# HKUST-Aerial-Robotics/ESVO

Hardware: AMD Instinct MI355X
Metric: mapped events/sec (stereo TS raster + block matching + LM depth refinement + fusion), events resident in HBM before the timed region; exactly K ticks between two synchronisations, i.e. including the fill and the drain of the two-deep tick pipeline (`sustained`: the same workload over 1600 ticks) (higher is better)
Workload: dtype f64

## Files before the change

### esvo_amd/csrc/api_core.hip

```cpp
#include "context.hpp"

namespace esvo_host {
thread_local std::string g_create_error;
}

namespace {

void invert3x3(const double* P, double* Kinv, double* Kinv_t) {
  const double a = P[0], b = P[1], cc = P[2], d = P[4], e = P[5], f = P[6], g = P[8], hh = P[9], i = P[10];
  const double det = a * (e * i - f * hh) - b * (d * i - f * g) + cc * (d * hh - e * g);
  const double id = 1.0 / det;
  Kinv[0] = (e * i - f * hh) * id; Kinv[1] = (cc * hh - b * i) * id; Kinv[2] = (b * f - cc * e) * id;
  Kinv[3] = (f * g - d * i) * id;  Kinv[4] = (a * i - cc * g) * id;  Kinv[5] = (cc * d - a * f) * id;
  Kinv[6] = (d * hh - e * g) * id; Kinv[7] = (b * g - a * hh) * id;  Kinv[8] = (a * e - b * d) * id;
  for (int r = 0; r < 3; ++r) Kinv_t[r] = (Kinv[r * 3 + 0] * P[3] + Kinv[r * 3 + 1] * P[7]) + Kinv[r * 3 + 2] * P[11];
}

int validate_params(const esvo_params_t* p, std::string& why) {
  if (p->ls_norm != ESVO_LSNORM_TDIST && p->ls_norm != ESVO_LSNORM_L2) { why = "LSnorm must be Tdist or l2 (DepthProblemSolver.cpp:121-131 exits on anything else)"; return ESVO_ERR_UNSUPPORTED; }
  if (p->bm_step < 1) { why = "BM_step must be >= 1"; return ESVO_ERR_INVALID_ARG; }
  if (p->patch_size_x < 1 || p->patch_size_x > 64 || p->patch_size_y < 1 || p->patch_size_y > 40) { why = "patch size must be within 1..64 x 1..40"; return ESVO_ERR_UNSUPPORTED; }
  if (p->median_blur_kernel_size < 0 || p->median_blur_kernel_size > 3) { why = "median_blur_kernel_size must be 0..3 (kernel 2k + 1)"; return ESVO_ERR_UNSUPPORTED; }
  if (p->max_event_queue_len < 0 || p->max_event_queue_len > TSQ_LMAX) { why = "max_event_queue_len must be 0 (one stamp per pixel) or 1..32"; return ESVO_ERR_UNSUPPORTED; }
  if (p->bm_max_disparity < p->bm_min_disparity || p->bm_min_disparity < 0) { why = "bad disparity range"; return ESVO_ERR_INVALID_ARG; }
// ... 25 lines not shown
  d.cost_thr = (p.residual_vis_threshold * p.residual_vis_threshold) * (double)(p.patch_size_x * p.patch_size_y);
  d.age_thr = p.age_vis_threshold;
  d.fusion_radius = p.fusion_radius;
  d.reg_radius = p.reg_radius; d.reg_min_nb = p.reg_min_neighbours; d.reg_min_close = p.reg_min_close_neighbours;
  d.num_threads = p.num_threads;
  d.ls_norm = p.ls_norm;
}

template <typename T>
hipError_t dalloc(T** p, size_t n) { return hipMalloc(reinterpret_cast<void**>(p), (n ? n : 1) * sizeof(T)); }

void set_compute_band(esvo_context* h) {
  const int halo = 2 + (h->prm.regularization ? h->prm.reg_radius : 0);
  h->dp.cband_y0 = std::max(0, h->dp.band_y0 - halo);
  h->dp.cband_y1 = std::min(h->H, h->dp.band_y1 + halo);
}

void release_routing(esvo_context* h) {
  for (int cam = 0; cam < 2; ++cam) {
    if (h->h_route_ev[cam]) hipHostFree(h->h_route_ev[cam]);
    h->h_route_ev[cam] = nullptr;
    h->route_cap[cam] = 0;
  }
  if (h->h_route_gidx) hipHostFree(h->h_route_gidx);
  h->h_route_gidx = nullptr;
}

}

extern "C" {
// ... 219 lines not shown
  CK(hipMalloc(reinterpret_cast<void**>(&h->d_map), map_buffer_bytes(npx)));
  CK(hipMalloc(reinterpret_cast<void**>(&h->d_map2), map_buffer_bytes(npx)));
  CK(hipMemset(h->d_map, 0, map_buffer_bytes(npx)));
  CK(hipMemset(h->d_map2, 0, map_buffer_bytes(npx)));
  h->d_map_cur = h->d_map;
  CK(dalloc(&h->d_owner_max, npx));
  CK(dalloc(&h->d_owner_min, npx));
  CK(dalloc(&h->d_own_w, E));
  CK(dalloc(&h->d_lkeep, E));
  h->codes_bytes = (E + 7) / 8 * 8;
  CK(dalloc(&h->d_codes, h->codes_bytes));
  CK(dalloc(&h->d_sel, E));
  CK(dalloc(&h->d_evmap, npx + 64));
  CK(dalloc(&h->d_reg_ab, npx));
  CK(dalloc(&h->d_reg_cd, npx));
  CK(dalloc(&h->d_exp_flags, npx));
  CK(dalloc(&h->d_exp_prefix, npx));
  CK(dalloc(&h->d_export, npx));
  CK(dalloc(&h->d_export_cell, npx));
  for (int i = 0; i < EV_N; ++i) CK(hipEventCreate(&h->evt[i]));
  if (h->tl_on) { CK(hipEventCreate(&h->tl_ref)); CK(hipEventRecord(h->tl_ref, h->stream)); CK(hipEventSynchronize(h->tl_ref)); }
  h->evt_ok = true;
  CK(hipEventCreateWithFlags(&h->evt_trk_read, hipEventDisableTiming));
  for (int cam = 0; cam < 2; ++cam) CK(hipEventCreateWithFlags(&h->evt_ingest[cam], hipEventDisableTiming));
  CK(hipHostMalloc(reinterpret_cast<void**>(&h->h_pose_pool), sizeof(double) * 16 * (size_t)h->max_poses * esvo_context::POSE_POOL));
  for (int i = 0; i < esvo_context::POSE_POOL; ++i) CK(hipEventCreate(&h->pool_evt[i]));
  h->pool_ok = true;
  for (int i = 0; i < 16; ++i) h->T_world_obs[i] = h->T_world_frame[i] = (i % 5 == 0) ? 1.0 : 0.0;
#undef CK
  *out = h;
// ... 4 lines not shown
  if (!h) return ESVO_OK;
  hipSetDevice(h->device);
  if (h->stream) hipStreamSynchronize(h->stream);
  if (h->stream_l) hipStreamSynchronize(h->stream_l);
  if (h->stream_l1) hipStreamSynchronize(h->stream_l1);
  if (h->stream_b) hipStreamSynchronize(h->stream_b);
  comm_release(h);
  em_release(h);
  void* ptrs[] = {h->d_lut, h->d_mask, h->d_fixmap[0], h->d_fixmap[1], h->d_sae[0], h->d_sae[1], h->d_raw, h->d_raw1, h->d_fwd_lut[0], h->d_fwd_lut[1], h->d_fwd_off[0], h->d_fwd_off[1],
                  h->d_fwd_src[0], h->d_fwd_src[1], h->d_fwd_val, h->d_ts[0],
                  h->d_ts[1], h->d_ring[0], h->d_ring[1], h->d_obs2[0][0], h->d_obs2[0][1], h->d_obs2[1][0], h->d_obs2[1][1], h->d_obs_tmp,
                  h->d_pose_T2[0], h->d_pose_T2[1], h->d_scan_tmp_b, h->d_cnt_b, h->d_tick_ev, h->d_match_slots, h->d_match_flags, h->d_match_prefix,
                  h->d_matches2[0], h->d_matches2[1], h->d_scan_tmp_l2[0], h->d_scan_tmp_l2[1], h->d_pt_slots2[0], h->d_pt_slots2[1], h->d_pt_flags2[0], h->d_pt_flags2[1], h->d_pt_prefix2[0], h->d_pt_prefix2[1], h->d_pts_tmp, h->d_stage[0], h->d_stage[1], h->d_counters2[0], h->d_counters2[1], h->d_scan_tmp,
                  h->d_win, h->d_frame_pose_T, h->d_fr_table, h->d_prop, h->d_tile_pts, h->d_tile_count, h->d_over_pts,
                  h->d_cell_count, h->d_cell_offset, h->d_cell_list, h->d_fuse_ctr, h->d_rec_ids, h->d_map, h->d_map2, h->d_owner_max, h->d_owner_min, h->d_exp_flags,
                  h->d_exp_prefix, h->d_export, h->d_export_cell, h->d_reg_ab, h->d_reg_cd, h->d_tsq[0], h->d_tsq[1], h->d_tsq_tcount, h->d_tsq_tlist, h->d_tsq_over, h->d_tsq_over_count, h->d_own_w, h->d_lkeep, h->d_codes, h->d_codes_send, h->d_codes_all, h->d_pts_send, h->d_pts_all, h->d_rank_kept,
                  h->d_sel, h->d_evmap, h->d_lm_fvec0, h->d_lm_fnorm0, h->d_lm_meta, h->d_lm_order, h->d_lm_hist, h->d_clk, h->d_ring_gidx, h->d_halo_viol, h->d_dn_flags, h->d_merge_a, h->d_merge_b, h->d_merge_plan, h->d_tsq_dup};
  for (void* p : ptrs) if (p) hipFree(p);
  if (h->h_counters) hipHostFree(h->h_counters);
  if (h->h_cnt_b) hipHostFree(h->h_cnt_b);
  if (h->h_pin) hipHostFree(h->h_pin);
  if (h->h_fr_table) hipHostFree(h->h_fr_table);
  if (h->evt_ok) for (int i = 0; i < EV_N; ++i) hipEventDestroy(h->evt[i]);
  if (h->pool_ok) for (int i = 0; i < esvo_context::POSE_POOL; ++i) hipEventDestroy(h->pool_evt[i]);
  if (h->h_pose_pool) hipHostFree(h->h_pose_pool);
  if (h->h_trk_ne) hipHostFree(h->h_trk_ne);
  if (h->h_trk_solve) hipHostFree(h->h_trk_solve);
  if (h->h_trk_xyz) hipHostFree(h->h_trk_xyz);
  release_routing(h);
  for (int cam = 0; cam < 2; ++cam) if (h->d_wire[cam]) hipFree(h->d_wire[cam]);
  if (h->evt_trk_read) hipEventDestroy(h->evt_trk_read);
// ... 118 lines not shown
    if (need > h->max_frames) FAIL(ESVO_ERR_CAPACITY, "fusion window (frames) exceeds the capacity fixed at esvo_create");
  }
  if (h->routed && (params->smooth_time_surface != h->prm.smooth_time_surface || params->median_blur_kernel_size != h->prm.median_blur_kernel_size ||
                    params->patch_size_y != h->prm.patch_size_y || params->denoising != h->prm.denoising || params->bm_updown))
    FAIL(ESVO_ERR_STATE, "the handle routes events by row (esvo_shard_set_routing): SmoothTimeSurface, median_blur_kernel_size, patch_size_Y and Denoising "
                         "fix the rows it renders and the events it keeps; esvo_reset + esvo_shard_set_routing to change them");
  esvo_params_t np = *params;
  np.max_events_per_tick = h->prm.max_events_per_tick;
  np.max_window_points = h->prm.max_window_points;
  np.max_poses_per_tick = h->prm.max_poses_per_tick;
  np.event_ring_capacity = h->prm.event_ring_capacity;
  if (np.max_event_queue_len != h->prm.max_event_queue_len) FAIL(ESVO_ERR_CAPACITY, "max_event_queue_len is fixed at esvo_create (the per-pixel queues are allocated there)");
  h->prm = np;
  fill_dev_params(h);
  set_compute_band(h);
  return ESVO_OK;
}

int esvo_set_stream(esvo_handle h, void* hip_stream) {
  if (!h) return ESVO_ERR_INVALID_ARG;
  API_LOCK(h);
  std::lock_guard<std::mutex> lp0(h->mu_push[0]), lp1(h->mu_push[1]);
  { int rcp = flush_pending_tick(h); if (rcp) return rcp; }
  HIPCHK(hipStreamSynchronize(h->stream));
  HIPCHK(hipStreamSynchronize(h->stream_l)); HIPCHK(hipStreamSynchronize(h->stream_l1));
  HIPCHK(hipStreamSynchronize(h->stream_b));
  if (h->own_stream && h->stream) hipStreamDestroy(h->stream);
  h->stream = reinterpret_cast<hipStream_t>(hip_stream);
  h->own_stream = false;
  return ESVO_OK;
// ... 105 lines not shown
```

### esvo_amd/csrc/api_map.hip

```cpp
#include <chrono>

#include "context.hpp"

namespace esvo_host {

u64 lower_bound_sec(const esvo_context* h, int cam, double t) {
  const auto& v = h->ts_host[cam];
  size_t lo = 0, hi = v.size();
  while (lo < hi) {
    size_t mid = (lo + hi) / 2;
    if (ns_to_sec(v[mid]) < t) lo = mid + 1; else hi = mid;
  }
  return h->ring_base[cam] + lo;
}
u64 ros_time_from_sec(double t) {
  long long sec64 = (long long)std::floor(t);
  u32 sec = (u32)sec64;
  u32 nsec = (u32)std::round((t - sec) * 1e9);
  sec += (nsec / 1000000000ul);
  nsec %= 1000000000ul;
  return (u64)sec * 1000000000ull + nsec;
}

int upload_poses(esvo_context* h, const uint64_t* pose_t_ns, const double* pose_T, size_t m, u32* d_zero_row = nullptr) {
// ... 351 lines not shown
  const int o = par * EV_BACK_STRIDE;
  const bool timed = h->stage_events_on;
  h->back_timed[par] = timed;
  if (timed) hipEventRecord(h->evt[EV_FU0 + o], sb);
  launch_fuse(a, h->dp, sb);
  if (timed) hipEventRecord(h->evt[EV_FU1 + o], sb);
  h->d_map_cur = h->d_map;
  h->map_id_bound = total * ((naive || h->dp.fusion_radius == 0) ? 4u : 9u);
  const bool do_clean = naive ? false : (h->prm.clean_requires_full_window ? (h->n_window_frames >= (size_t)h->prm.max_fusion_frames) : true);
  if (do_clean) launch_clean(h->d_map, h->dp, sb);
  if (timed) hipEventRecord(h->evt[EV_CL1 + o], sb);
  if (h->prm.regularization && !naive) {
    launch_reg_view(h->d_map, h->d_map2, h->d_owner_max, h->d_owner_min, h->d_reg_ab, h->d_reg_cd, h->d_cnt_b + 7, h->dp, sb);
    const u64 band_cells = (u64)std::max(h->dp.band_y1 - h->dp.band_y0, 1) * (u64)h->W;
    const bool sparse = h->reg_sparse_forced >= 0 ? h->reg_sparse_forced == 1 : (u64)h->stats.last_map_size * 10u < band_cells;
    launch_reg_apply(h->d_map, h->d_map2, h->d_owner_max, h->d_owner_min, h->d_reg_ab, h->d_reg_cd, h->d_cnt_b + 7, h->dp, sb, sparse);
    h->d_map_cur = h->d_map2;
  }
  HIPCHK(hipMemcpyAsync(h->h_cnt_b + 8 * par, h->d_cnt_b, sizeof(u32) * 8, hipMemcpyDeviceToHost, sb));
  if (h->routed) HIPCHK(hipMemcpyAsync(h->h_cnt_b + 8 * 3 + par, h->d_halo_viol, sizeof(u32), hipMemcpyDeviceToHost, sb));
  hipEventRecord(h->evt[EV_RG1 + o], sb);
  for (int e : tail_ev) if (e >= 0) hipEventRecord(h->evt[e], sb);
  HIPCHK(hipGetLastError());
  h->back_pending[par] = true;
  return ESVO_OK;
}

int export_map(esvo_context* h, std::vector<esvo_depth_point_t>& out, std::vector<u32>* cells) {
  launch_map_compact(h->d_map_cur, h->d_exp_flags, h->d_exp_prefix, h->d_cnt_b + 5, h->d_scan_tmp_b, h->d_export,
                     h->d_export_cell, h->dp, h->stream_b);
  int rc = read_counters_b(h, 2, true);
// ... 1653 lines not shown
```

### esvo_amd/csrc/common.hpp

```cpp
#pragma once

#include <hip/hip_runtime.h>
#include <stdint.h>

#include "../../include/esvo_hip.h"

#define ESVO_WAVE 64

#include <cstdlib>
#include <cstring>
inline const char* esvo_dev_switch(const char* name) {
  const char* on = std::getenv("ESVO_DEV_SWITCHES");
  return (on && std::strcmp(on, "1") == 0) ? std::getenv(name) : nullptr;
}

namespace esvo {

typedef unsigned long long u64;
typedef unsigned int u32;

struct CamConst {
  double P[12];
  double Kinv[9];
  double Kinv_t[3];
// ... 301 lines not shown
  u32 lds_cap;
  u32 pmax_plus1;
  u32* d_total;
  MapCell* map;
  u32* d_num_fusion;
  u32* n_touched;
  int naive;
  u32* owner_max;
  u32* owner_min;
  u32* n_reg_elems;
};
void launch_fuse(const FuseArgs& a, const DevParams& p, hipStream_t s);
void launch_clean(MapCell* map, const DevParams& p, hipStream_t s);
void launch_reg_view(const MapCell* map_in, MapCell* map_out, u32* owner_max, u32* owner_min, double2* ab, double2* cd,
                     u32* n_elems, const DevParams& p, hipStream_t s);
void launch_reg_apply(const MapCell* map_in, MapCell* map_out, const u32* owner_max, const u32* owner_min, const double2* ab,
                      const double2* cd, u32* n_elems, const DevParams& p, hipStream_t s, bool sparse = false);
struct SgmScratch {
  uint8_t *sobL, *rawL, *sobR, *rawR;
  int16_t* vol[6];
  int16_t *d1, *d1b;
  u32* d2key;
};
void launch_sgbm(const uint8_t* left, const uint8_t* right, const SgmScratch& s, int16_t* disp, int W, int H, hipStream_t st);
void launch_sgm_points(const esvo_event_t* ring, u64 first, u64 cap, u32 n, const float2* lut, const int16_t* disp, DevPoint* slots,
                       u32* flags, const DevParams& p, hipStream_t st);
void launch_sgm_tick_points(const esvo_event_t* ev, u64 first, u64 cap, int reverse, u32 n, const float2* lut, const int16_t* disp,
                            DevPoint* slots, u32* flags, u32* cnt, const DevParams& p, hipStream_t st);
void launch_sgm_naive(const DevPoint* pts, u32 n, const double* d_T_frame_obs, u32* owner, u32* pair_flags, u32* pair_rank, u32* d_total,
                      u32* scan_tmp, MapCell* map, const DevParams& p, hipStream_t st);
void launch_debug_image(const MapCell* map, u32* owner, uint8_t* bgr, const uint8_t* jet, int type, double max_range,
                        double min_range, double thr1, double thr2, const DevParams& p, hipStream_t s);
// ... 7 lines not shown
```

### esvo_amd/csrc/context.hpp

```cpp
#pragma once
#include <algorithm>
#include <array>
#include <atomic>
#include <chrono>
#include <cmath>
#include <cstdio>
#include <cstdlib>
#include <cstring>
#include <deque>
#include <mutex>
#include <string>
#include <vector>

#include "common.hpp"

using namespace esvo;

enum { EV_SC0 = 0, EV_SC1, EV_R1, EV_SC0b, EV_SC1b, EV_R1b, EV_FRAME,
       EV_T0, EV_BM0, EV_BM1, EV_S1, EV_LM0, EV_LM1, EV_S2, EV_CNT, EV_STG, EV_A1, EV_T0b, EV_BM0b, EV_BM1b, EV_S1b, EV_LM0b, EV_LM1b, EV_S2b, EV_CNTb, EV_STGb, EV_A1b,
       EV_FU0, EV_FU1, EV_CL1, EV_RG1, EV_POSE, EV_FU0b, EV_FU1b, EV_CL1b, EV_RG1b, EV_POSEb, EV_N };
constexpr int EV_BACK_STRIDE = EV_FU0b - EV_FU0;
constexpr int EV_FRONT_STRIDE = EV_T0b - EV_T0;
constexpr int EV_TS_STRIDE = EV_SC0b - EV_SC0;

// ... 241 lines not shown
  bool tick_pending = false;
  u64 committed_t_ns = 0;
  int tsq_len = 0;
  u64* d_tsq[2] = {nullptr, nullptr};
  u32* d_tsq_tcount = nullptr;
  uint4* d_tsq_tlist = nullptr;
  uint4* d_tsq_over = nullptr;
  u32* d_tsq_over_count = nullptr;
  u32 tsq_tcap = 0;
  static constexpr u64 TSQ_ROUND = 1ull << 20;
  u64 sh_first = 0;
  u64 sh_first_prev = 0;
  u64 em_guard_lo[2] = {~0ull, ~0ull};
  double2* d_reg_ab = nullptr;
  double2* d_reg_cd = nullptr;
  double T_world_frame[16];
  u32* d_exp_flags = nullptr;
  u32* d_exp_prefix = nullptr;
  esvo_depth_point_t* d_export = nullptr;
  u32* d_export_cell = nullptr;
  u32 map_id_bound = 0;
  float* d_cloud_xyz[2] = {nullptr, nullptr};
  int cloud_cur = -1;
  size_t cloud_n = 0;
  u64 cloud_t_ns = 0;
  u32* d_cloud_ids = nullptr;
  size_t cloud_id_cap = 0;
  u32* d_cloud_scan = nullptr;
  u32* d_cloud_cnt = nullptr;
  u32* h_cloud_cnt = nullptr;
// ... 146 lines not shown
```

### esvo_amd/csrc/dev_hooks.hpp

```cpp
#pragma once
#if defined(LM_STATS) || defined(REG_STATS) || defined(ESVO_PERTURB_ONE_ULP)
#include "../../tools/dev_hooks/hooks_impl.hpp"
#endif
#ifndef LM_STATS
#define DEV_LM_EVAL(pr) do {} while (0)
#define DEV_LM_SHORTCUT(pr) do {} while (0)
#define DEV_LM_PROBLEM_FIELDS
#define DEV_LM_SET_SLOT(pr, s) do {} while (0)
#define DEV_LM_FIRST_EVAL_KNZ(pr, knz) do {} while (0)
#define DEV_LM_SCALE_ITER(pr) do {} while (0)
#define DEV_LM_JAC_DECL
#define DEV_LM_JAC_PASS(pr, active, x) do {} while (0)
#endif
#ifndef ESVO_PERTURB_ONE_ULP
#define DEV_PERTURB_POINT(o, s) do {} while (0)
#endif
#ifndef REG_STATS
#define DEV_REG_DECL
#define DEV_REG_BLOCK_BEGIN() do {} while (0)
#define DEV_REG_ROW_BEGIN(nclose)
#define DEV_REG_ROW_END(nclose) do {} while (0)
#define DEV_REG_BLOCK_END(lane, wv) do {} while (0)
#define DEV_REG_DONE(t, lane, nclose) do {} while (0)
#endif
```

### esvo_amd/csrc/kernels_fuse.hip

```cpp
#include <algorithm>
#include <type_traits>
#define DEV_HOOKS_FUSE_TU
#include "common.hpp"
#include "dev_hooks.hpp"
#include "fdiv.hpp"
#include "scan.hpp"

namespace esvo {

#ifndef BACK_WAVES
#define BACK_WAVES 6
#endif
#ifndef FUSE_WAVES
#define FUSE_WAVES 1
#endif

__device__ inline bool boundaryCheck(double x, double y, int W, int H) {
  return !(x < 0 || x >= (double)W || y < 0 || y >= (double)H);
}

__device__ inline bool fusion_cell(u32 prow, u32 pcol, int k, int radius, int W, int H, int& row, int& col) {
  int dy, dx;
  if (radius == 0) { dy = k >> 1; dx = k & 1; }
  else { dy = k / 3 - 1; dx = k % 3 - 1; }
// ... 624 lines not shown
  }
  const u64 am = __ballot(alive);
  if (n_elems && (threadIdx.x & 63) == 0 && am) atomicAdd(n_elems, (u32)__popcll(am));
}

#define REG_TX 64
#ifndef REG_TY
#define REG_TY 8
#endif
#ifndef REG_RB
#define REG_RB 4
#endif
#define REG_MARGIN 1
#define REG_MAXW 128
static_assert((REG_TX * REG_TY) % 64 == 0 && REG_TX == 64, "a wave is a tile row");
template <int RT, bool SPARSE = false>
__global__ void __launch_bounds__(REG_TX * REG_TY, BACK_WAVES) reg_apply_kernel(const MapCell* __restrict__ map, MapCell* __restrict__ out,
                                                                    const u32* __restrict__ owner_max,
                                                                    const u32* __restrict__ owner_min,
                                                                    const double2* __restrict__ ab,
                                                                    const double2* __restrict__ cd, DevParams p, u32* __restrict__ n_elems) {
  constexpr int NW = REG_TY;
  constexpr int UNITS = 4 * REG_RB;
  constexpr int UPW = (UNITS + NW - 1) / NW;
  __shared__ double2 s_ab[2][REG_RB][REG_MAXW];
  __shared__ double2 s_cd[2][REG_RB][REG_MAXW];
  __shared__ u64 s_vb[2][REG_RB][2];
  __shared__ u32 s_elem[REG_TX * REG_TY];
  __shared__ u32 s_wcount[REG_TY + 1];
  const int t = threadIdx.x, lane = t & 63, wv = t >> 6;
  const int tiles_x = (p.W + REG_TX - 1) / REG_TX;
  const int tile_c0 = (int)(blockIdx.x % tiles_x) * REG_TX, tile_r0 = (int)(blockIdx.x / tiles_x) * REG_TY;
  const int R = RT > 0 ? RT : p.reg_radius, Wn = 2 * R + 1;
  const int cr = tile_r0 + wv, cc = tile_c0 + lane;
  bool alive = false;
  if (cr < p.H && cc < p.W && cr >= p.band_y0 && cr < p.band_y1) alive = (map_flags(map, p.W * p.H)[cr * p.W + cc] & CELL_ALIVE) != 0;
  const u64 am = __ballot(alive);
  if (lane == 0) s_wcount[wv] = (u32)__popcll(am);
  __syncthreads();
  u32 base = 0, n_el = 0;
  for (int w = 0; w < REG_TY; ++w) { if (w < wv) base += s_wcount[w]; n_el += s_wcount[w]; }
  if (n_el == 0) return;
  if (t == 0) atomicAdd(n_elems, n_el);
  if (alive) s_elem[base + (u32)__popcll(am & ((1ull << lane) - 1ull))] = (u32)(cr * p.W + cc);
  __syncthreads();
  const bool has = (u32)t < n_el;
  int cell = 0, row = 0, col = 0;
  double inv = -1.0, sd_self2 = 0.0;
  u32 seq = 0;
  if (has) {
    cell = (int)s_elem[t];
    const MapCell& c = map[cell];
    row = (int)c.row; col = (int)c.col;
    inv = c.inv_depth;
    sd_self2 = 2.0 * sqrt(c.variance);
    seq = c.seq;
  }
  const u32 b = (u32)row * (u32)p.W + (u32)col;
  const bool owner = has && owner_max[b] == seq + 1u;
  bool scan = owner && inv > -1e-6 && row >= R && col >= R;
  const int sc0 = tile_c0 - REG_MARGIN - R, sr0 = tile_r0 - REG_MARGIN - R;
  const int sw = REG_TX + 2 * (R + REG_MARGIN), sh = REG_TY + 2 * (R + REG_MARGIN);
  const int off = col - R - sc0;
  bool slow = scan && (off < 0 || off + Wn > sw || row - R < sr0 || row + R >= sr0 + sh);
  if (slow) scan = false;
  const u64 wmask = (Wn >= 64) ? ~0ull : ((1ull << Wn) - 1ull);
  u32 nb = 0, nclose = 0;
  double nu_post = 0, inv_post = 0, s2_post = 0, nu_div = 0;
  Recip rnu = make_recip(1.0);
  bool first = true;
  auto fuse_step = [&](double inv_obs, double nu_obs, double s2_obs) {
    if (first) {
      first = false;
      nu_post = nu_obs; inv_post = inv_obs; s2_post = s2_obs;
      nu_div = nu_post + 1;
      rnu = make_recip(nu_div);
      return;
    }
    const double nu_prior = nu_post, inv_prior = inv_post, s2_prior = s2_post;
    nu_post = (nu_obs < nu_prior) ? nu_obs : nu_prior;
    if (nu_post + 1 != nu_div) { nu_div = nu_post + 1; rnu = make_recip(nu_div); }
    const double ssum = s2_obs + s2_prior;
    const Recip rsum = make_recip(ssum);
    const double a1 = s2_obs * inv_prior + s2_prior * inv_obs;
    const double dd = inv_prior - inv_obs;
    const double a2 = dd * dd;
    const double pp = s2_prior * s2_obs;
    const double q1 = div_fast(a1, rsum);
    const double a3 = nu_post + div_fast(a2, rsum);
    const double a4 = div_fast(a3, rnu) * pp;
    const double q4 = div_fast(a4, rsum);
    const bool ok = (int)rnu.fast & (int)fdiv_ok_b4(ssum, a1, a2, a3, a4);
    if (ok) {
      inv_post = q1;
      s2_post = q4;
    } else {
      inv_post = a1 / ssum;
      s2_post = ((nu_post + a2 / ssum) / (nu_post + 1) * pp) / ssum;
    }
  };
  const double nan = __longlong_as_double(0x7ff8000000000000ll);
  double2 ld[UPW];
  const int n_blk = (sh + REG_RB - 1) / REG_RB;
  auto fetch_block = [&](int k) {
#pragma unroll
    for (int j = 0; j < UPW; ++j) {
      const int u = wv + NW * j;
      ld[j] = make_double2(nan, nan);
      if (u < UNITS && k < n_blk) {
        const int r = u >> 2, a = (u >> 1) & 1, hf = u & 1;
        const int y = k * REG_RB + r, sj = hf * 64 + lane;
        const int gy = sr0 + y, gx = sc0 + sj;
        if (sj < sw && y < sh && gy >= 0 && gy < p.H && gx >= 0 && gx < p.W) ld[j] = (a ? cd : ab)[gy * p.W + gx];
      }
    }
  };
  auto store_block = [&](int buf) {
#pragma unroll
    for (int j = 0; j < UPW; ++j) {
      const int u = wv + NW * j;
      if (u < UNITS) {
        const int r = u >> 2, a = (u >> 1) & 1, hf = u & 1;
        const int sj = hf * 64 + lane;
        (a ? s_cd : s_ab)[buf][r][sj] = ld[j];
        if (!a) {
          const u64 vm = __ballot(sj < sw && ld[j].x == ld[j].x);
          if (lane == 0) s_vb[buf][r][hf] = vm;
        }
      }
    }
  };
  DEV_REG_DECL
  fetch_block(0);
  store_block(0);
  fetch_block(1);
  __syncthreads();
  for (int k = 0; k < n_blk; ++k) {
    const int buf = k & 1;
    DEV_REG_BLOCK_BEGIN();
#pragma unroll 1
    for (int r = 0; r < REG_RB; ++r) {
      const int gy = sr0 + k * REG_RB + r;
      DEV_REG_ROW_BEGIN(nclose)
      if (scan && gy >= row - R && gy <= row + R) {
        const u64 w0 = s_vb[buf][r][0], w1 = s_vb[buf][r][1];
        u64 bits = (off < 64) ? (w0 >> off) : 0ull;
        if (off > 0 && off < 64) bits |= w1 << (64 - off);
        if (off >= 64) bits = w1 >> (off - 64);
        bits &= wmask;
        nb += (u32)__popcll(bits);
        u32 cm2[2] = {0u, 0u};
        if (bits) {
          u32 lo = 0, hi = 0;
          const double2* tap = &s_ab[buf][r][off];
          if constexpr (SPARSE) {
#pragma unroll 1
            for (int half = 0; half < 2; ++half) {
              u32 m = half ? (u32)(bits >> 32) : (u32)bits;
              u32 acc = 0;
              while (m) {
                const int kk = __builtin_ctz(m);
                m &= m - 1u;
                const double2 q = tap[32 * half + kk];
                acc |= (fabs(inv - q.x) < fmax(sd_self2, q.y)) ? (1u << kk) : 0u;
              }
              if (half) hi = acc; else lo = acc;
            }
          } else if (RT > 0) {
#pragma unroll
            for (int dc = 0; dc < 2 * RT + 1; ++dc) {
              const double2 q = tap[dc];
              const bool close = fabs(inv - q.x) < fmax(sd_self2, q.y);
              if (dc < 32) lo |= close ? (1u << dc) : 0u; else hi |= close ? (1u << (dc - 32)) : 0u;
            }
          } else {
            for (int dc = 0; dc < Wn; ++dc) {
              const double2 q = tap[dc];
              const bool close = fabs(inv - q.x) < fmax(sd_self2, q.y);
              if (dc < 32) lo |= close ? (1u << dc) : 0u; else hi |= close ? (1u << (dc - 32)) : 0u;
            }
          }
          cm2[0] = lo; cm2[1] = hi;
        }
        nclose += (u32)__popc(cm2[0]) + (u32)__popc(cm2[1]);
#pragma unroll 1
        for (int half = 0; half < 2; ++half) {
          u32 m = half ? cm2[1] : cm2[0];
          const int o2 = off + 32 * half;
          while (m) {
            const int kk = __builtin_ctz(m);
            m &= m - 1u;
            const double2 qa = s_ab[buf][r][o2 + kk], qc = s_cd[buf][r][o2 + kk];
            fuse_step(qa.x, qc.x, qc.y);
          }
        }
      }
      DEV_REG_ROW_END(nclose);
    }
    DEV_REG_BLOCK_END(lane, wv);
    if (k + 1 < n_blk) store_block(buf ^ 1);
    fetch_block(k + 2);
    __syncthreads();
  }
  DEV_REG_DONE(t, lane, nclose);
  if (slow) {
    for (int r = row - R; r <= row + R && r < p.H; ++r)
      for (int c2 = col - R; c2 <= col + R && c2 < p.W; ++c2) {
        const double2 q = ab[r * p.W + c2];
        if (!(q.x == q.x)) continue;
        nb++;
        const double diff = fabs(inv - q.x);
        if (diff < sd_self2 || diff < q.y) {
          nclose++;
          const double2 qc = cd[r * p.W + c2];
          fuse_step(q.x, qc.x, qc.y);
        }
      }
  }
  if (!has) return;
  u32* of = map_flags(out, p.W * p.H);
  if (!owner) { of[cell] = 0; return; }
  MapCell c = map[cell];
  if (c.inv_depth > -1e-6)
    c.inv_depth = (nb > (u32)p.reg_min_nb && nclose > (u32)p.reg_min_close) ? inv_post : -1.0;
  c.seq = owner_min[b];
  out[cell] = c;
  of[cell] = CELL_ALIVE | CELL_GRID;
}

__global__ void __launch_bounds__(256) reg_apply_l2_kernel(const MapCell* __restrict__ map, MapCell* __restrict__ out,
                                                           const u32* __restrict__ owner_max, const u32* __restrict__ owner_min,
                                                           const double2* __restrict__ ab, const double2* __restrict__ cd, DevParams p) {
  const int cell = blockIdx.x * blockDim.x + threadIdx.x;
  if (cell >= p.W * p.H) return;
  { const int r0 = cell / p.W; if (r0 < p.band_y0 || r0 >= p.band_y1) return; }
  if (!(map_flags(map, p.W * p.H)[cell] & CELL_ALIVE)) return;
  MapCell c = map[cell];
  u32* of = map_flags(out, p.W * p.H);
  const int row = (int)c.row, col = (int)c.col, R = p.reg_radius;
  const u32 b = (u32)row * (u32)p.W + (u32)col;
  if (owner_max[b] != c.seq + 1u) { of[cell] = 0; return; }
  if (c.inv_depth > -1e-6) {
// ... 23 lines not shown
    c.inv_depth = set ? mean : -1.0;
  }
  c.seq = owner_min[b];
  out[cell] = c;
  of[cell] = CELL_ALIVE | CELL_GRID;
}

void launch_reg_view(const MapCell* map_in, MapCell* map_out, u32* owner_max, u32* owner_min, double2* ab, double2* cd,
                     u32* n_elems, const DevParams& p, hipStream_t s) {
  const int ncell = p.W * p.H;
  const int nb = (ncell + 255) / 256;
  if (p.ls_norm != ESVO_LSNORM_L2) n_elems = nullptr;
  hipLaunchKernelGGL(reg_view_kernel, dim3(nb), dim3(256), 0, s, map_in, map_out, ab, cd, owner_max, owner_min, n_elems, ncell, p.W,
                     p.band_y0, p.band_y1, p.cband_y0, p.cband_y1, p.ls_norm == ESVO_LSNORM_L2 ? 1 : 0);
}
void launch_reg_apply(const MapCell* map_in, MapCell* map_out, const u32* owner_max, const u32* owner_min, const double2* ab,
                      const double2* cd, u32* n_elems, const DevParams& p, hipStream_t s, bool sparse) {
  if (p.ls_norm == ESVO_LSNORM_L2) {
    const int ncell = p.W * p.H;
    hipLaunchKernelGGL(reg_apply_l2_kernel, dim3((ncell + 255) / 256), dim3(256), 0, s, map_in, map_out, owner_max, owner_min, ab, cd, p);
    return;
  }
  const int tiles_x = (p.W + REG_TX - 1) / REG_TX;
  const int ty0 = p.band_y0 / REG_TY, ty1 = (p.band_y1 + REG_TY - 1) / REG_TY;
  if (ty1 <= ty0) return;
  const int tiles_y = (p.H + REG_TY - 1) / REG_TY;
  const dim3 grid(tiles_x * tiles_y), block(REG_TX * REG_TY);
  if (sparse) {
    if (p.reg_radius == 20) hipLaunchKernelGGL((reg_apply_kernel<20, true>), grid, block, 0, s, map_in, map_out, owner_max, owner_min, ab, cd, p, n_elems);
    else if (p.reg_radius == 5) hipLaunchKernelGGL((reg_apply_kernel<5, true>), grid, block, 0, s, map_in, map_out, owner_max, owner_min, ab, cd, p, n_elems);
    else hipLaunchKernelGGL((reg_apply_kernel<0, true>), grid, block, 0, s, map_in, map_out, owner_max, owner_min, ab, cd, p, n_elems);
    return;
  }
  if (p.reg_radius == 20) hipLaunchKernelGGL(reg_apply_kernel<20>, grid, block, 0, s, map_in, map_out, owner_max, owner_min, ab, cd, p, n_elems);
  else if (p.reg_radius == 5) hipLaunchKernelGGL(reg_apply_kernel<5>, grid, block, 0, s, map_in, map_out, owner_max, owner_min, ab, cd, p, n_elems);
  else hipLaunchKernelGGL(reg_apply_kernel<0>, grid, block, 0, s, map_in, map_out, owner_max, owner_min, ab, cd, p, n_elems);
}

__global__ void __launch_bounds__(256) map_flags_kernel(const MapCell* __restrict__ map, u32* __restrict__ flags, int ncell, int W,
                                                        int band0, int band1) {
  const int cell = blockIdx.x * blockDim.x + threadIdx.x;
  if (cell >= ncell) return;
  const int row = cell / W;
  flags[cell] = (row >= band0 && row < band1 && (map_flags(map, ncell)[cell] & CELL_ALIVE)) ? 1u : 0u;
}
__global__ void __launch_bounds__(256) map_export_kernel(const MapCell* __restrict__ map, const u32* __restrict__ flags,
                                                         const u32* __restrict__ prefix, esvo_depth_point_t* __restrict__ out,
                                                         u32* __restrict__ out_cell, int ncell) {
  const int cell = blockIdx.x * blockDim.x + threadIdx.x;
  if (cell >= ncell || !flags[cell]) return;
  const MapCell& c = map[cell];
// ... 21 lines not shown
```

Measured before the change: 154.4 million.

## Split regularisation into mask scan plus load-balanced sorted fusion walk kernel

The regularisation apply kernel now only computes per-row close-neighbour bitmasks and writes them to a per-cell record buffer. It then buckets cells by neighbour count into class/slice lists. A new turn kernel prefix-sums the class counts, and a walk kernel assigns one lane per cell, ordered by workload class, to run the sequential fusion steps with a small prefetch queue. This targets wave divergence in the serial fuse loop, where cells with very different neighbour counts shared a wave and the cd tile also had to be staged in LDS. The cost is extra kernel launches, global record traffic and more scratch memory.

```diff
diff --git a/esvo_amd/csrc/api_core.hip b/esvo_amd/csrc/api_core.hip
--- a/esvo_amd/csrc/api_core.hip
+++ b/esvo_amd/csrc/api_core.hip
@@ -63,6 +63,31 @@
   const int halo = 2 + (h->prm.regularization ? h->prm.reg_radius : 0);
   h->dp.cband_y0 = std::max(0, h->dp.band_y0 - halo);
   h->dp.cband_y1 = std::min(h->H, h->dp.band_y1 + halo);
+}
+
+hipError_t reg_walk_alloc(esvo_context* h) {
+  RegWalk& w = h->reg_walk;
+  if (!h->prm.regularization) return hipSuccess;
+  const size_t npx = (size_t)h->W * h->H;
+  hipError_t e;
+  if (!w.list) {
+    w.cap = (u32)npx;
+    w.slice_cap = reg_slice_cap(h->W, h->H);
+    if ((e = dalloc(&w.list, (size_t)REG_NB * REG_SLICES * w.slice_cap)) != hipSuccess) return e;
+    if ((e = dalloc(&w.class_count, 2 * (size_t)REG_NB * REG_SLICES + 1)) != hipSuccess) return e;
+    if ((e = hipMemset(w.class_count, 0, sizeof(u32) * (2 * (size_t)REG_NB * REG_SLICES + 1))) != hipSuccess) return e;
+    w.class_total = w.class_count + REG_NB * REG_SLICES;
+  }
+  const u32 words = reg_rec_words(h->prm.reg_radius);
+  if (words > h->reg_rec_alloc_words) {
+    if (h->stream_b && (e = hipStreamSynchronize(h->stream_b)) != hipSuccess) return e;
+    if (w.rec) { hipFree(w.rec); w.rec = nullptr; h->reg_rec_alloc_words = 0; }
+    if ((e = dalloc(&w.rec, npx * words)) != hipSuccess) return e;
+    h->reg_rec_alloc_words = words;
+  }
+  w.rec_words = words;
+  w.class_width = reg_class_width(h->prm.reg_radius);
+  return hipSuccess;
 }
 
 void release_routing(esvo_context* h) {
@@ -312,6 +337,7 @@
   CK(dalloc(&h->d_evmap, npx + 64));
   CK(dalloc(&h->d_reg_ab, npx));
   CK(dalloc(&h->d_reg_cd, npx));
+  CK(reg_walk_alloc(h));
   CK(dalloc(&h->d_exp_flags, npx));
   CK(dalloc(&h->d_exp_prefix, npx));
   CK(dalloc(&h->d_export, npx));
@@ -346,7 +372,7 @@
                   h->d_matches2[0], h->d_matches2[1], h->d_scan_tmp_l2[0], h->d_scan_tmp_l2[1], h->d_pt_slots2[0], h->d_pt_slots2[1], h->d_pt_flags2[0], h->d_pt_flags2[1], h->d_pt_prefix2[0], h->d_pt_prefix2[1], h->d_pts_tmp, h->d_stage[0], h->d_stage[1], h->d_counters2[0], h->d_counters2[1], h->d_scan_tmp,
                   h->d_win, h->d_frame_pose_T, h->d_fr_table, h->d_prop, h->d_tile_pts, h->d_tile_count, h->d_over_pts,
                   h->d_cell_count, h->d_cell_offset, h->d_cell_list, h->d_fuse_ctr, h->d_rec_ids, h->d_map, h->d_map2, h->d_owner_max, h->d_owner_min, h->d_exp_flags,
-                  h->d_exp_prefix, h->d_export, h->d_export_cell, h->d_reg_ab, h->d_reg_cd, h->d_tsq[0], h->d_tsq[1], h->d_tsq_tcount, h->d_tsq_tlist, h->d_tsq_over, h->d_tsq_over_count, h->d_own_w, h->d_lkeep, h->d_codes, h->d_codes_send, h->d_codes_all, h->d_pts_send, h->d_pts_all, h->d_rank_kept,
+                  h->d_exp_prefix, h->d_export, h->d_export_cell, h->d_reg_ab, h->d_reg_cd, h->reg_walk.rec, h->reg_walk.list, h->reg_walk.class_count, h->d_tsq[0], h->d_tsq[1], h->d_tsq_tcount, h->d_tsq_tlist, h->d_tsq_over, h->d_tsq_over_count, h->d_own_w, h->d_lkeep, h->d_codes, h->d_codes_send, h->d_codes_all, h->d_pts_send, h->d_pts_all, h->d_rank_kept,
                   h->d_sel, h->d_evmap, h->d_lm_fvec0, h->d_lm_fnorm0, h->d_lm_meta, h->d_lm_order, h->d_lm_hist, h->d_clk, h->d_ring_gidx, h->d_halo_viol, h->d_dn_flags, h->d_merge_a, h->d_merge_b, h->d_merge_plan, h->d_tsq_dup};
   for (void* p : ptrs) if (p) hipFree(p);
   if (h->h_counters) hipHostFree(h->h_counters);
@@ -495,6 +521,7 @@
   h->prm = np;
   fill_dev_params(h);
   set_compute_band(h);
+  HIPCHK(reg_walk_alloc(h));
   return ESVO_OK;
 }
 
diff --git a/esvo_amd/csrc/api_map.hip b/esvo_amd/csrc/api_map.hip
--- a/esvo_amd/csrc/api_map.hip
+++ b/esvo_amd/csrc/api_map.hip
@@ -389,7 +389,7 @@
     launch_reg_view(h->d_map, h->d_map2, h->d_owner_max, h->d_owner_min, h->d_reg_ab, h->d_reg_cd, h->d_cnt_b + 7, h->dp, sb);
     const u64 band_cells = (u64)std::max(h->dp.band_y1 - h->dp.band_y0, 1) * (u64)h->W;
     const bool sparse = h->reg_sparse_forced >= 0 ? h->reg_sparse_forced == 1 : (u64)h->stats.last_map_size * 10u < band_cells;
-    launch_reg_apply(h->d_map, h->d_map2, h->d_owner_max, h->d_owner_min, h->d_reg_ab, h->d_reg_cd, h->d_cnt_b + 7, h->dp, sb, sparse);
+    launch_reg_apply(h->d_map, h->d_map2, h->d_owner_max, h->d_owner_min, h->d_reg_ab, h->d_reg_cd, h->d_cnt_b + 7, h->dp, sb, sparse, h->reg_walk);
     h->d_map_cur = h->d_map2;
   }
   HIPCHK(hipMemcpyAsync(h->h_cnt_b + 8 * par, h->d_cnt_b, sizeof(u32) * 8, hipMemcpyDeviceToHost, sb));
diff --git a/esvo_amd/csrc/common.hpp b/esvo_amd/csrc/common.hpp
--- a/esvo_amd/csrc/common.hpp
+++ b/esvo_amd/csrc/common.hpp
@@ -339,8 +339,23 @@
 void launch_clean(MapCell* map, const DevParams& p, hipStream_t s);
 void launch_reg_view(const MapCell* map_in, MapCell* map_out, u32* owner_max, u32* owner_min, double2* ab, double2* cd,
                      u32* n_elems, const DevParams& p, hipStream_t s);
+#define REG_NB 16
+#define REG_SLICES 16
+struct RegWalk {
+  u32* rec;
+  u32 rec_words;
+  u32 cap;
+  u32* list;
+  u32 slice_cap;
+  u32 class_width;
+  u32* class_count;
+  u32* class_total;
+};
+__host__ __device__ inline u32 reg_rec_words(int radius) { return 2u + 2u * (2u * (u32)radius + 1u); }
+__host__ __device__ inline u32 reg_class_width(int radius) { const u32 wn = 2u * (u32)radius + 1u; const u32 w = wn * wn / 70u; return w < 4u ? 4u : w; }
+u32 reg_slice_cap(int W, int H);
 void launch_reg_apply(const MapCell* map_in, MapCell* map_out, const u32* owner_max, const u32* owner_min, const double2* ab,
-                      const double2* cd, u32* n_elems, const DevParams& p, hipStream_t s, bool sparse = false);
+                      const double2* cd, u32* n_elems, const DevParams& p, hipStream_t s, bool sparse, const RegWalk& w);
 struct SgmScratch {
   uint8_t *sobL, *rawL, *sobR, *rawR;
   int16_t* vol[6];
diff --git a/esvo_amd/csrc/context.hpp b/esvo_amd/csrc/context.hpp
--- a/esvo_amd/csrc/context.hpp
+++ b/esvo_amd/csrc/context.hpp
@@ -279,6 +279,8 @@
   u64 em_guard_lo[2] = {~0ull, ~0ull};
   double2* d_reg_ab = nullptr;
   double2* d_reg_cd = nullptr;
+  RegWalk reg_walk{};
+  u32 reg_rec_alloc_words = 0;
   double T_world_frame[16];
   u32* d_exp_flags = nullptr;
   u32* d_exp_prefix = nullptr;
diff --git a/esvo_amd/csrc/dev_hooks.hpp b/esvo_amd/csrc/dev_hooks.hpp
--- a/esvo_amd/csrc/dev_hooks.hpp
+++ b/esvo_amd/csrc/dev_hooks.hpp
@@ -16,10 +16,6 @@
 #define DEV_PERTURB_POINT(o, s) do {} while (0)
 #endif
 #ifndef REG_STATS
-#define DEV_REG_DECL
-#define DEV_REG_BLOCK_BEGIN() do {} while (0)
-#define DEV_REG_ROW_BEGIN(nclose)
-#define DEV_REG_ROW_END(nclose) do {} while (0)
-#define DEV_REG_BLOCK_END(lane, wv) do {} while (0)
-#define DEV_REG_DONE(t, lane, nclose) do {} while (0)
+#define DEV_REG_SCAN_DONE(walk, nclose) do {} while (0)
+#define DEV_REG_WALK_DONE(lane, has, n) do {} while (0)
 #endif
diff --git a/esvo_amd/csrc/kernels_fuse.hip b/esvo_amd/csrc/kernels_fuse.hip
--- a/esvo_amd/csrc/kernels_fuse.hip
+++ b/esvo_amd/csrc/kernels_fuse.hip
@@ -662,62 +662,11 @@
 #define REG_MARGIN 1
 #define REG_MAXW 128
 static_assert((REG_TX * REG_TY) % 64 == 0 && REG_TX == 64, "a wave is a tile row");
-template <int RT, bool SPARSE = false>
-__global__ void __launch_bounds__(REG_TX * REG_TY, BACK_WAVES) reg_apply_kernel(const MapCell* __restrict__ map, MapCell* __restrict__ out,
-                                                                    const u32* __restrict__ owner_max,
-                                                                    const u32* __restrict__ owner_min,
-                                                                    const double2* __restrict__ ab,
-                                                                    const double2* __restrict__ cd, DevParams p, u32* __restrict__ n_elems) {
-  constexpr int NW = REG_TY;
-  constexpr int UNITS = 4 * REG_RB;
-  constexpr int UPW = (UNITS + NW - 1) / NW;
-  __shared__ double2 s_ab[2][REG_RB][REG_MAXW];
-  __shared__ double2 s_cd[2][REG_RB][REG_MAXW];
-  __shared__ u64 s_vb[2][REG_RB][2];
-  __shared__ u32 s_elem[REG_TX * REG_TY];
-  __shared__ u32 s_wcount[REG_TY + 1];
-  const int t = threadIdx.x, lane = t & 63, wv = t >> 6;
-  const int tiles_x = (p.W + REG_TX - 1) / REG_TX;
-  const int tile_c0 = (int)(blockIdx.x % tiles_x) * REG_TX, tile_r0 = (int)(blockIdx.x / tiles_x) * REG_TY;
-  const int R = RT > 0 ? RT : p.reg_radius, Wn = 2 * R + 1;
-  const int cr = tile_r0 + wv, cc = tile_c0 + lane;
-  bool alive = false;
-  if (cr < p.H && cc < p.W && cr >= p.band_y0 && cr < p.band_y1) alive = (map_flags(map, p.W * p.H)[cr * p.W + cc] & CELL_ALIVE) != 0;
-  const u64 am = __ballot(alive);
-  if (lane == 0) s_wcount[wv] = (u32)__popcll(am);
-  __syncthreads();
-  u32 base = 0, n_el = 0;
-  for (int w = 0; w < REG_TY; ++w) { if (w < wv) base += s_wcount[w]; n_el += s_wcount[w]; }
-  if (n_el == 0) return;
-  if (t == 0) atomicAdd(n_elems, n_el);
-  if (alive) s_elem[base + (u32)__popcll(am & ((1ull << lane) - 1ull))] = (u32)(cr * p.W + cc);
-  __syncthreads();
-  const bool has = (u32)t < n_el;
-  int cell = 0, row = 0, col = 0;
-  double inv = -1.0, sd_self2 = 0.0;
-  u32 seq = 0;
-  if (has) {
-    cell = (int)s_elem[t];
-    const MapCell& c = map[cell];
-    row = (int)c.row; col = (int)c.col;
-    inv = c.inv_depth;
-    sd_self2 = 2.0 * sqrt(c.variance);
-    seq = c.seq;
-  }
-  const u32 b = (u32)row * (u32)p.W + (u32)col;
-  const bool owner = has && owner_max[b] == seq + 1u;
-  bool scan = owner && inv > -1e-6 && row >= R && col >= R;
-  const int sc0 = tile_c0 - REG_MARGIN - R, sr0 = tile_r0 - REG_MARGIN - R;
-  const int sw = REG_TX + 2 * (R + REG_MARGIN), sh = REG_TY + 2 * (R + REG_MARGIN);
-  const int off = col - R - sc0;
-  bool slow = scan && (off < 0 || off + Wn > sw || row - R < sr0 || row + R >= sr0 + sh);
-  if (slow) scan = false;
-  const u64 wmask = (Wn >= 64) ? ~0ull : ((1ull << Wn) - 1ull);
-  u32 nb = 0, nclose = 0;
+struct RegFuse {
   double nu_post = 0, inv_post = 0, s2_post = 0, nu_div = 0;
   Recip rnu = make_recip(1.0);
   bool first = true;
-  auto fuse_step = [&](double inv_obs, double nu_obs, double s2_obs) {
+  __device__ inline void step(double inv_obs, double nu_obs, double s2_obs) {
     if (first) {
       first = false;
       nu_post = nu_obs; inv_post = inv_obs; s2_post = s2_obs;
@@ -746,7 +695,62 @@
       inv_post = a1 / ssum;
       s2_post = ((nu_post + a2 / ssum) / (nu_post + 1) * pp) / ssum;
     }
-  };
+  }
+};
+template <int RT, bool SPARSE = false>
+__global__ void __launch_bounds__(REG_TX * REG_TY, BACK_WAVES) reg_apply_kernel(const MapCell* __restrict__ map, MapCell* __restrict__ out,
+                                                                    const u32* __restrict__ owner_max,
+                                                                    const u32* __restrict__ owner_min,
+                                                                    const double2* __restrict__ ab,
+                                                                    const double2* __restrict__ cd, DevParams p, u32* __restrict__ n_elems, RegWalk w) {
+  constexpr int NW = REG_TY;
+  constexpr int UNITS = 2 * REG_RB;
+  constexpr int UPW = (UNITS + NW - 1) / NW;
+  __shared__ double2 s_ab[2][REG_RB][REG_MAXW];
+  __shared__ u64 s_vb[2][REG_RB][2];
+  __shared__ u32 s_elem[REG_TX * REG_TY];
+  __shared__ u32 s_wcount[REG_TY + 1];
+  __shared__ u32 s_hist[REG_NB], s_hbase[REG_NB];
+  const int t = threadIdx.x, lane = t & 63, wv = t >> 6;
+  const int tiles_x = (p.W + REG_TX - 1) / REG_TX;
+  const int tile_c0 = (int)(blockIdx.x % tiles_x) * REG_TX, tile_r0 = (int)(blockIdx.x / tiles_x) * REG_TY;
+  const int R = RT > 0 ? RT : p.reg_radius, Wn = 2 * R + 1;
+  const int cr = tile_r0 + wv, cc = tile_c0 + lane;
+  bool alive = false;
+  if (cr < p.H && cc < p.W && cr >= p.band_y0 && cr < p.band_y1) alive = (map_flags(map, p.W * p.H)[cr * p.W + cc] & CELL_ALIVE) != 0;
+  const u64 am = __ballot(alive);
+  if (lane == 0) s_wcount[wv] = (u32)__popcll(am);
+  if (t < REG_NB) s_hist[t] = 0;
+  __syncthreads();
+  u32 base = 0, n_el = 0;
+  for (int w = 0; w < REG_TY; ++w) { if (w < wv) base += s_wcount[w]; n_el += s_wcount[w]; }
+  if (n_el == 0) return;
+  if (t == 0) s_wcount[REG_TY] = atomicAdd(n_elems, n_el);
+  if (alive) s_elem[base + (u32)__popcll(am & ((1ull << lane) - 1ull))] = (u32)(cr * p.W + cc);
+  __syncthreads();
+  const bool has = (u32)t < n_el;
+  int cell = 0, row = 0, col = 0;
+  double inv = -1.0, sd_self2 = 0.0;
+  u32 seq = 0;
+  if (has) {
+    cell = (int)s_elem[t];
+    const MapCell& c = map[cell];
+    row = (int)c.row; col = (int)c.col;
+    inv = c.inv_depth;
+    sd_self2 = 2.0 * sqrt(c.variance);
+    seq = c.seq;
+  }
+  const u32 b = (u32)row * (u32)p.W + (u32)col;
+  const bool owner = has && owner_max[b] == seq + 1u;
+  bool scan = owner && inv > -1e-6 && row >= R && col >= R;
+  const int sc0 = tile_c0 - REG_MARGIN - R, sr0 = tile_r0 - REG_MARGIN - R;
+  const int sw = REG_TX + 2 * (R + REG_MARGIN), sh = REG_TY + 2 * (R + REG_MARGIN);
+  const int off = col - R - sc0;
+  const u32 slot = s_wcount[REG_TY] + (u32)t;
+  bool slow = scan && (off < 0 || off + Wn > sw || row - R < sr0 || row + R >= sr0 + sh || slot >= w.cap);
+  if (slow) scan = false;
+  const u64 wmask = (Wn >= 64) ? ~0ull : ((1ull << Wn) - 1ull);
+  u32 nb = 0, nclose = 0;
   const double nan = __longlong_as_double(0x7ff8000000000000ll);
   double2 ld[UPW];
   const int n_blk = (sh + REG_RB - 1) / REG_RB;
@@ -756,10 +760,10 @@
       const int u = wv + NW * j;
       ld[j] = make_double2(nan, nan);
       if (u < UNITS && k < n_blk) {
-        const int r = u >> 2, a = (u >> 1) & 1, hf = u & 1;
+        const int r = u >> 1, hf = u & 1;
         const int y = k * REG_RB + r, sj = hf * 64 + lane;
         const int gy = sr0 + y, gx = sc0 + sj;
-        if (sj < sw && y < sh && gy >= 0 && gy < p.H && gx >= 0 && gx < p.W) ld[j] = (a ? cd : ab)[gy * p.W + gx];
+        if (sj < sw && y < sh && gy >= 0 && gy < p.H && gx >= 0 && gx < p.W) ld[j] = ab[gy * p.W + gx];
       }
     }
   };
@@ -768,28 +772,23 @@
     for (int j = 0; j < UPW; ++j) {
       const int u = wv + NW * j;
       if (u < UNITS) {
-        const int r = u >> 2, a = (u >> 1) & 1, hf = u & 1;
+        const int r = u >> 1, hf = u & 1;
         const int sj = hf * 64 + lane;
-        (a ? s_cd : s_ab)[buf][r][sj] = ld[j];
-        if (!a) {
-          const u64 vm = __ballot(sj < sw && ld[j].x == ld[j].x);
-          if (lane == 0) s_vb[buf][r][hf] = vm;
-        }
+        s_ab[buf][r][sj] = ld[j];
+        const u64 vm = __ballot(sj < sw && ld[j].x == ld[j].x);
+        if (lane == 0) s_vb[buf][r][hf] = vm;
       }
     }
   };
-  DEV_REG_DECL
   fetch_block(0);
   store_block(0);
   fetch_block(1);
   __syncthreads();
   for (int k = 0; k < n_blk; ++k) {
     const int buf = k & 1;
-    DEV_REG_BLOCK_BEGIN();
 #pragma unroll 1
     for (int r = 0; r < REG_RB; ++r) {
       const int gy = sr0 + k * REG_RB + r;
-      DEV_REG_ROW_BEGIN(nclose)
       if (scan && gy >= row - R && gy <= row + R) {
         const u64 w0 = s_vb[buf][r][0], w1 = s_vb[buf][r][1];
         u64 bits = (off < 64) ? (w0 >> off) : 0ull;
@@ -819,7 +818,9 @@
             for (int dc = 0; dc < 2 * RT + 1; ++dc) {
               const double2 q = tap[dc];
               const bool close = fabs(inv - q.x) < fmax(sd_self2, q.y);
-              if (dc < 32) lo |= close ? (1u << dc) : 0u; else hi |= close ? (1u << (dc - 32)) : 0u;
+              u32 c01 = close ? 1u : 0u;
+              asm volatile("" : "+v"(c01));
+              if (dc < 32) lo |= c01 << dc; else hi |= c01 << (dc - 32);
             }
           } else {
             for (int dc = 0; dc < Wn; ++dc) {
@@ -831,27 +832,16 @@
           cm2[0] = lo; cm2[1] = hi;
         }
         nclose += (u32)__popc(cm2[0]) + (u32)__popc(cm2[1]);
-#pragma unroll 1
-        for (int half = 0; half < 2; ++half) {
-          u32 m = half ? cm2[1] : cm2[0];
-          const int o2 = off + 32 * half;
-          while (m) {
-            const int kk = __builtin_ctz(m);
-            m &= m - 1u;
-            const double2 qa = s_ab[buf][r][o2 + kk], qc = s_cd[buf][r][o2 + kk];
-            fuse_step(qa.x, qc.x, qc.y);
-          }
-        }
-      }
-      DEV_REG_ROW_END(nclose);
-    }
-    DEV_REG_BLOCK_END(lane, wv);
+        *reinterpret_cast<uint2*>(w.rec + (size_t)slot * w.rec_words + (2 + 2 * (gy - (row - R)))) = make_uint2(cm2[0], cm2[1]);
+      }
+    }
     if (k + 1 < n_blk) store_block(buf ^ 1);
     fetch_block(k + 2);
     __syncthreads();
   }
-  DEV_REG_DONE(t, lane, nclose);
+  double inv_plain = 0.0;
   if (slow) {
+    RegFuse f;
     for (int r = row - R; r <= row + R && r < p.H; ++r)
       for (int c2 = col - R; c2 <= col + R && c2 < p.W; ++c2) {
         const double2 q = ab[r * p.W + c2];
@@ -861,19 +851,138 @@
         if (diff < sd_self2 || diff < q.y) {
           nclose++;
           const double2 qc = cd[r * p.W + c2];
-          fuse_step(q.x, qc.x, qc.y);
+          f.step(q.x, qc.x, qc.y);
         }
       }
-  }
-  if (!has) return;
+    inv_plain = f.inv_post;
+  }
+  cell = has ? (int)s_elem[t] : 0;
+  const u32 slot_e = s_wcount[REG_TY] + (u32)t;
+  const bool keep = nb > (u32)p.reg_min_nb && nclose > (u32)p.reg_min_close;
+  const bool walk = scan && keep;
+  DEV_REG_SCAN_DONE(walk, nclose);
+  u32 cls = 0, rank = 0;
+  if (walk) {
+    cls = nclose / w.class_width;
+    cls = cls < REG_NB - 1u ? cls : REG_NB - 1u;
+    rank = atomicAdd(&s_hist[cls], 1u);
+    *reinterpret_cast<uint2*>(w.rec + (size_t)slot_e * w.rec_words) = make_uint2((u32)cell, nclose);
+  }
+  __syncthreads();
+  const u32 slice = blockIdx.x % REG_SLICES;
+  if (t < REG_NB && s_hist[t]) s_hbase[t] = atomicAdd(&w.class_count[t * REG_SLICES + slice], s_hist[t]);
+  __syncthreads();
+  if (walk) w.list[((size_t)cls * REG_SLICES + slice) * w.slice_cap + s_hbase[cls] + rank] = slot_e;
+  if (!has || walk) return;
   u32* of = map_flags(out, p.W * p.H);
   if (!owner) { of[cell] = 0; return; }
   MapCell c = map[cell];
   if (c.inv_depth > -1e-6)
-    c.inv_depth = (nb > (u32)p.reg_min_nb && nclose > (u32)p.reg_min_close) ? inv_post : -1.0;
-  c.seq = owner_min[b];
+    c.inv_depth = keep ? inv_plain : -1.0;
+  c.seq = owner_min[(u32)row * (u32)p.W + (u32)col];
   out[cell] = c;
   of[cell] = CELL_ALIVE | CELL_GRID;
+}
+
+#define REG_NSEG (REG_NB * REG_SLICES)
+__global__ void __launch_bounds__(REG_NSEG) reg_turn_kernel(RegWalk w) {
+  __shared__ u32 lds[REG_NSEG / ESVO_WAVE];
+  const u32 seg = threadIdx.x;
+  const u32 cls = REG_NB - 1u - seg / REG_SLICES, slc = seg % REG_SLICES;
+  const u32 c = w.class_count[cls * REG_SLICES + slc];
+  w.class_count[cls * REG_SLICES + slc] = 0;
+  u32 tot;
+  const u32 ex = block_excl_scan<REG_NSEG / ESVO_WAVE>(c, &tot, lds);
+  w.class_total[seg] = ex;
+  if (seg == 0) w.class_total[REG_NSEG] = tot;
+}
+
+#define REG_WALK_B 64
+#define REG_AHEAD 4
+__global__ void __launch_bounds__(REG_WALK_B) reg_walk_kernel(const MapCell* __restrict__ map, MapCell* __restrict__ out,
+                                                              const u32* __restrict__ owner_min, const double2* __restrict__ ab,
+                                                              const double2* __restrict__ cd, DevParams p, RegWalk w) {
+  extern __shared__ u32 s_walk[];
+  const u32 total = w.class_total[REG_NSEG];
+  if (blockIdx.x * REG_WALK_B >= total) return;
+  const int lane = threadIdx.x;
+  u32* s_seg = s_walk;
+  for (u32 i = (u32)lane; i <= REG_NSEG; i += REG_WALK_B) s_seg[i] = w.class_total[i];
+  __syncthreads();
+  const int R = p.reg_radius, Wn = 2 * R + 1, nw = 2 * Wn;
+  u32* sm = s_walk + (REG_NSEG + 1) + lane * (nw + 1);
+  const u32 t = blockIdx.x * REG_WALK_B + (u32)lane;
+  const int ncell = p.W * p.H;
+  bool has = t < total;
+  u32 cell = 0, n = 0;
+  int r0 = 0, c0 = 0;
+  if (has) {
+    u32 lo = 0, hi = REG_NSEG;
+    while (hi - lo > 1) { const u32 mid = (lo + hi) >> 1; if (s_seg[mid] <= t) lo = mid; else hi = mid; }
+    const u32 cls = REG_NB - 1u - lo / REG_SLICES, slc = lo % REG_SLICES;
+    const u32 slot = w.list[((size_t)cls * REG_SLICES + slc) * w.slice_cap + (t - s_seg[lo])];
+    has = slot < w.cap;
+    const uint4* rec = reinterpret_cast<const uint4*>(w.rec + (size_t)(has ? slot : 0u) * w.rec_words);
+    const uint4 h0 = rec[0];
+    cell = h0.x;
+    has = has && cell < (u32)ncell;
+    if (has) {
+      const MapCell& c = map[cell];
+      const int row = (int)c.row, col = (int)c.col;
+      r0 = row - R; c0 = col - R;
+      has = r0 >= 0 && c0 >= 0 && row < p.H && col < p.W;
+    }
+    if (has) {
+      const int rows_in = p.H - r0 < Wn ? p.H - r0 : Wn;
+      const int cols_in = p.W - c0;
+      const u64 cmask = cols_in >= 64 ? ~0ull : ((1ull << cols_in) - 1ull);
+      const u32 m_lo = (u32)cmask, m_hi = (u32)(cmask >> 32);
+      auto put = [&](int j, u32 m) {
+        m &= (j & 1) ? m_hi : m_lo;
+        if ((j >> 1) >= rows_in) m = 0;
+        sm[j] = m;
+        n += (u32)__popc(m);
+      };
+      put(0, h0.z); put(1, h0.w);
+      for (int q = 1; q < (int)(w.rec_words >> 2); ++q) {
+        const uint4 v = rec[q];
+        const int j = 4 * q - 2;
+        put(j, v.x); put(j + 1, v.y); put(j + 2, v.z); put(j + 3, v.w);
+      }
+    }
+  }
+  int g_i = -1;
+  u32 g_m = 0;
+  auto next_tap = [&]() -> int {
+    while (g_m == 0 && g_i + 1 < nw) { ++g_i; g_m = sm[g_i]; }
+    if (g_m == 0) return -1;
+    const int kk = __builtin_ctz(g_m);
+    g_m &= g_m - 1u;
+    return (r0 + (g_i >> 1)) * p.W + c0 + 32 * (g_i & 1) + kk;
+  };
+  RegFuse f;
+  double q_inv[REG_AHEAD], q_nu[REG_AHEAD], q_s2[REG_AHEAD];
+  auto fetch = [&](int j) {
+    const int idx = next_tap();
+    if (idx >= 0) { q_inv[j] = ab[idx].x; const double2 qc = cd[idx]; q_nu[j] = qc.x; q_s2[j] = qc.y; }
+  };
+#pragma unroll
+  for (int j = 0; j < REG_AHEAD; ++j) { q_inv[j] = q_nu[j] = q_s2[j] = 0.0; if ((u32)j < n) fetch(j); }
+  for (u32 i = 0; i < n; i += REG_AHEAD) {
+#pragma unroll
+    for (int j = 0; j < REG_AHEAD; ++j)
+      if (i + (u32)j < n) {
+        f.step(q_inv[j], q_nu[j], q_s2[j]);
+        if (i + (u32)j + REG_AHEAD < n) fetch(j);
+      }
+  }
+  DEV_REG_WALK_DONE(lane, has, n);
+  if (!has) return;
+  MapCell c = map[cell];
+  c.inv_depth = f.inv_post;
+  c.seq = owner_min[c.row * (u32)p.W + c.col];
+  out[cell] = c;
+  map_flags(out, ncell)[cell] = CELL_ALIVE | CELL_GRID;
 }
 
 __global__ void __launch_bounds__(256) reg_apply_l2_kernel(const MapCell* __restrict__ map, MapCell* __restrict__ out,
@@ -927,8 +1036,22 @@
   hipLaunchKernelGGL(reg_view_kernel, dim3(nb), dim3(256), 0, s, map_in, map_out, ab, cd, owner_max, owner_min, n_elems, ncell, p.W,
                      p.band_y0, p.band_y1, p.cband_y0, p.cband_y1, p.ls_norm == ESVO_LSNORM_L2 ? 1 : 0);
 }
+u32 reg_slice_cap(int W, int H) {
+  const u32 n_tiles = (u32)((W + REG_TX - 1) / REG_TX) * (u32)((H + REG_TY - 1) / REG_TY);
+  return (n_tiles + REG_SLICES - 1) / REG_SLICES * (REG_TX * REG_TY);
+}
+static void launch_reg_walk(const MapCell* map_in, MapCell* map_out, const u32* owner_min, const double2* ab, const double2* cd,
+                            const DevParams& p, hipStream_t s, const RegWalk& w) {
+  hipLaunchKernelGGL(reg_turn_kernel, dim3(1), dim3(REG_NSEG), 0, s, w);
+  const u32 band_cells = (u32)std::max(p.band_y1 - p.band_y0, 0) * (u32)p.W;
+  const u32 lanes = std::min(band_cells, w.cap);
+  if (lanes == 0) return;
+  const size_t lds = sizeof(u32) * ((REG_NSEG + 1) + (size_t)REG_WALK_B * (2 * (2 * p.reg_radius + 1) + 1));
+  hipLaunchKernelGGL(reg_walk_kernel, dim3((lanes + REG_WALK_B - 1) / REG_WALK_B), dim3(REG_WALK_B), lds, s, map_in, map_out, owner_min, ab, cd,
+                     p, w);
+}
 void launch_reg_apply(const MapCell* map_in, MapCell* map_out, const u32* owner_max, const u32* owner_min, const double2* ab,
-                      const double2* cd, u32* n_elems, const DevParams& p, hipStream_t s, bool sparse) {
+                      const double2* cd, u32* n_elems, const DevParams& p, hipStream_t s, bool sparse, const RegWalk& w) {
   if (p.ls_norm == ESVO_LSNORM_L2) {
     const int ncell = p.W * p.H;
     hipLaunchKernelGGL(reg_apply_l2_kernel, dim3((ncell + 255) / 256), dim3(256), 0, s, map_in, map_out, owner_max, owner_min, ab, cd, p);
@@ -940,14 +1063,16 @@
   const int tiles_y = (p.H + REG_TY - 1) / REG_TY;
   const dim3 grid(tiles_x * tiles_y), block(REG_TX * REG_TY);
   if (sparse) {
-    if (p.reg_radius == 20) hipLaunchKernelGGL((reg_apply_kernel<20, true>), grid, block, 0, s, map_in, map_out, owner_max, owner_min, ab, cd, p, n_elems);
-    else if (p.reg_radius == 5) hipLaunchKernelGGL((reg_apply_kernel<5, true>), grid, block, 0, s, map_in, map_out, owner_max, owner_min, ab, cd, p, n_elems);
-    else hipLaunchKernelGGL((reg_apply_kernel<0, true>), grid, block, 0, s, map_in, map_out, owner_max, owner_min, ab, cd, p, n_elems);
+    if (p.reg_radius == 20) hipLaunchKernelGGL((reg_apply_kernel<20, true>), grid, block, 0, s, map_in, map_out, owner_max, owner_min, ab, cd, p, n_elems, w);
+    else if (p.reg_radius == 5) hipLaunchKernelGGL((reg_apply_kernel<5, true>), grid, block, 0, s, map_in, map_out, owner_max, owner_min, ab, cd, p, n_elems, w);
+    else hipLaunchKernelGGL((reg_apply_kernel<0, true>), grid, block, 0, s, map_in, map_out, owner_max, owner_min, ab, cd, p, n_elems, w);
+    launch_reg_walk(map_in, map_out, owner_min, ab, cd, p, s, w);
     return;
   }
-  if (p.reg_radius == 20) hipLaunchKernelGGL(reg_apply_kernel<20>, grid, block, 0, s, map_in, map_out, owner_max, owner_min, ab, cd, p, n_elems);
-  else if (p.reg_radius == 5) hipLaunchKernelGGL(reg_apply_kernel<5>, grid, block, 0, s, map_in, map_out, owner_max, owner_min, ab, cd, p, n_elems);
-  else hipLaunchKernelGGL(reg_apply_kernel<0>, grid, block, 0, s, map_in, map_out, owner_max, owner_min, ab, cd, p, n_elems);
+  if (p.reg_radius == 20) hipLaunchKernelGGL(reg_apply_kernel<20>, grid, block, 0, s, map_in, map_out, owner_max, owner_min, ab, cd, p, n_elems, w);
+  else if (p.reg_radius == 5) hipLaunchKernelGGL(reg_apply_kernel<5>, grid, block, 0, s, map_in, map_out, owner_max, owner_min, ab, cd, p, n_elems, w);
+  else hipLaunchKernelGGL(reg_apply_kernel<0>, grid, block, 0, s, map_in, map_out, owner_max, owner_min, ab, cd, p, n_elems, w);
+  launch_reg_walk(map_in, map_out, owner_min, ab, cd, p, s, w);
 }
 
 __global__ void __launch_bounds__(256) map_flags_kernel(const MapCell* __restrict__ map, u32* __restrict__ flags, int ncell, int W,
```

New measurement: 120.9 million. 21.7% lower.
